# fumiama/Retrieval-based-Voice-Conversion-WebUI

Measured on AMD Instinct MI355X. Metric: real-time factor (audio-sec/wall-sec), 48 kHz v2, 10 s clips, retrieval + NSF-HiFi-GAN decode, higher is better.
Workload: dtype fp16 MFMA operands + fp16 inter-stage streams (ResBlock outputs, ups output of stages 1-3), fp32 accumulate / in-block residual; fp32 MFMA prefilter + fp64 verified IVF distances; 1 GPU; BASELINE configs[1]: v2/48k, 1 x 10 s clip(s) per GPU, T=1198 frames, 599 queries/clip, IVF 10000x768 nlist=256 nprobe=1 k=8 index_rate=0.75; hipgraph=True, index_blob_bytes=32376576, launcher=single process

## Files before the change

retrieval-based-voice-conversion-webui_amd/csrc/nsf.hip:

```cpp
#include <algorithm>
#include <atomic>
#include <cmath>
#include <functional>
#include <memory>
#include <string>
#include <unordered_map>

#include "common.hpp"
#include "nsf_kernels.hpp"
#include "conv_pack.hpp"
#include "rb_stream.hpp"

namespace rvcmi {

thread_local std::string g_last_error;
void set_error(const char* fmt, ...) {
    char buf[1024];
    va_list ap;
    va_start(ap, fmt);
    vsnprintf(buf, sizeof(buf), fmt, ap);
    va_end(ap);
    g_last_error = buf;
}

// ... 133 lines not shown
        s.rb[j].resize(nd);
        for (int m = 0; m < nd; ++m) {
            const int d = cfg->resblock_dilation_sizes[j][m];
            const std::string base = "resblocks." + std::to_string(n);
            const int C = s.cout;
            for (int which = 0; which < 2; ++which) {
                const std::string nm = base + (which ? ".convs2." : ".convs1.") + std::to_string(m);
                const rvcmi_tensor& w = wm.get(nm + ".weight", {C, C, k});
                const rvcmi_tensor& b = wm.get(nm + ".bias", {C});
                const int dil = which ? 1 : d;
                int nt = k, off = -((k * dil - dil) / 2);
                const float* wd = w.data;
                ConvLayer& L2 = which ? s.rb[j][m].second : s.rb[j][m].first;
                build_conv(L2, C, C, 1, &nt, &off, dil,
                           [=](int co, int ci, int, int tap) { return wd[((size_t)co * C + ci) * k + tap]; }, b.data, op);
            }
        }
    }
}

static void nsf_create(const rvcmi_nsf_config* cfg, const rvcmi_tensor* weights, int n_weights, int device, int max_B,
                       int max_T, rvcmi_nsf** out) {
    if (!cfg || !out || (!weights && n_weights)) RVCMI_FAIL(RVCMI_ERR_INVALID, "null argument");
    if (cfg->n_ups < 1 || cfg->n_ups > RVCMI_MAX_UPS || cfg->n_resblock_kernels < 1 ||
        cfg->n_resblock_kernels > RVCMI_MAX_RB)
        RVCMI_FAIL(RVCMI_ERR_INVALID, "bad stage counts");
    if (cfg->operand < 0 || cfg->operand > 2) RVCMI_FAIL(RVCMI_ERR_INVALID, "bad operand type %d", cfg->operand);
    if (max_B < 1 || max_T < 1) RVCMI_FAIL(RVCMI_ERR_INVALID, "max_B/max_T must be positive");
    HIP_CHECK(hipSetDevice(device));
    set_lds_limits();
    rb_stream_prepare();

    std::unique_ptr<rvcmi_nsf> h(new rvcmi_nsf());
    h->opt.load_env({"RB_STREAM", "NO_RB_SPLIT", "POST_DMA", "POST_DBG", "DBG", "Y_F16", "X0_F16", "X0_F16_NOSTREAM"});
    rb_stream_load_env(h->opt);
    h->cfg = *cfg;
    h->device = device;
    h->max_B = max_B;
    h->max_T = max_T;
    const int op = cfg->operand;
    WeightMap wm;
    for (int i = 0; i < n_weights; ++i) wm.m[weights[i].name] = &weights[i];

    const int C0 = cfg->upsample_initial_channel, inter = cfg->inter_channels;
    h->C0 = C0;
    {
        const rvcmi_tensor& w = wm.get("conv_pre.weight", {C0, inter, 7});
        const rvcmi_tensor& b = wm.get("conv_pre.bias", {C0});
        const float* wd = w.data;
        int nt = 7, off = -3;
        build_conv(h->pre, inter, C0, 1, &nt, &off, 1,
                   [=](int co, int ci, int, int tap) { return wd[((size_t)co * inter + ci) * 7 + tap]; }, b.data, op);
    }
    if (cfg->gin_channels) {
        const rvcmi_tensor& w = wm.get("cond.weight", {C0, cfg->gin_channels, 1});
        const rvcmi_tensor& b = wm.get("cond.bias", {C0});
        upload(h->cond_w, std::vector<float>(w.data, w.data + (size_t)C0 * cfg->gin_channels));
        upload(h->cond_b, std::vector<float>(b.data, b.data + C0));
    }
    if (cfg->use_f0) {
        h->lin_w = wm.get("m_source.l_linear.weight", {1, 1}).data[0];
        h->lin_b = wm.get("m_source.l_linear.bias", {1}).data[0];
    }
    int upp = 1;
    for (int i = 0; i < cfg->n_ups; ++i) upp *= cfg->upsample_rates[i];
    h->upp = upp;

// ... 224 lines not shown
#define RBF32_OCC 2
#endif
template <int C> struct RbFullGeom;
#ifndef RBF64_NWV
#define RBF64_NWV 8
#endif
#if RBF64_NWV == 8
template <> struct RbFullGeom<64> { static constexpr int MI = 2, NJ = 2, KG = 4, OCC = 2, NWV = 8; };
#else
template <> struct RbFullGeom<64> { static constexpr int MI = 2, NJ = 3, KG = 4, OCC = 1, NWV = 4; };
#endif
#ifndef RBF32_NWV
#define RBF32_NWV 4
#endif
template <> struct RbFullGeom<32> { static constexpr int MI = 1, NJ = RBF32_NJ, KG = 4, OCC = RBF32_OCC, NWV = RBF32_NWV; };
template <> struct RbFullGeom<16> { static constexpr int MI = 1, NJ = RBF32_NJ, KG = 4, OCC = RBF32_OCC, NWV = RBF32_NWV; };
static int rbf_rows(int C) { return C == 64 ? RbFullGeom<64>::NWV * 32 * RbFullGeom<64>::NJ : RBF32_NWV * 32 * RBF32_NJ; }
template <int C>
constexpr int rbf_nb() { return RbFullGeom<C>::NWV == 8 ? 2 : 3; }
template <typename OpT, int C>
static void launch_rbf_inst(const RbFullArgs& ra, int tiles, int nj, int B, hipStream_t st) {
    using G = RbFullGeom<C>;
    constexpr int R = G::NWV * 32 * G::NJ;
    const size_t smem = (size_t)(R + 2 * RBF_G + R + 2 * RBF_G2) * Tile<C>::STRIDE + 3 * 2 * 32 * G::MI * 4 + 512;
    hipLaunchKernelGGL((k_rb_full<OpT, C, G::MI, G::NJ, G::KG, rbf_nb<C>(), G::OCC, G::NWV>), dim3(tiles, nj, B), dim3(64 * G::NWV), smem, st, ra);
}
constexpr int RBF64S_NJ = 2, RBF64S_NWV = 4, RBF64S_ROWS = RBF64S_NWV * 32 * RBF64S_NJ;
template <typename OpT, int C>
static void launch_rbf_small(const RbFullArgs& ra, int tiles, int nj, int B, hipStream_t st) {
    constexpr int R = RBF64S_ROWS, MI = C == 64 ? 2 : 1, OCCS = C == 64 ? 1 : 2;
    const size_t smem = (size_t)(R + 2 * RBF_G + R + 2 * RBF_G2) * Tile<C>::STRIDE + 3 * 2 * 32 * MI * 4 + 512;
    hipLaunchKernelGGL((k_rb_full<OpT, C, MI, RBF64S_NJ, 4, 3, OCCS, RBF64S_NWV>), dim3(tiles, nj, B), dim3(64 * RBF64S_NWV), smem, st, ra);
}
template <typename OpT>
static void launch_rbf_t(int C, const RbFullArgs& ra, int tiles, int nj, int B, hipStream_t st, bool small64) {
    if (small64 && C == 64) return launch_rbf_small<OpT, 64>(ra, tiles, nj, B, st);
    if (small64 && C == 32) return launch_rbf_small<OpT, 32>(ra, tiles, nj, B, st);
    switch (C) {
        case 64: return launch_rbf_inst<OpT, 64>(ra, tiles, nj, B, st);
        case 32: return launch_rbf_inst<OpT, 32>(ra, tiles, nj, B, st);
        case 16: return launch_rbf_inst<OpT, 16>(ra, tiles, nj, B, st);
        default: RVCMI_FAIL(RVCMI_ERR_INVALID, "fused resblock: unsupported channel count %d", C);
    }
}
template <typename OpT>
static void set_lds_rbf() {
#define RBF_ATTR(C_)                                                                                                        \
    HIP_CHECK(hipFuncSetAttribute(reinterpret_cast<const void*>(&k_rb_full<OpT, C_, RbFullGeom<C_>::MI, RbFullGeom<C_>::NJ, RbFullGeom<C_>::KG, rbf_nb<C_>(), RbFullGeom<C_>::OCC, RbFullGeom<C_>::NWV>), \
                                  hipFuncAttributeMaxDynamicSharedMemorySize, 160 * 1024));
    RBF_ATTR(64) RBF_ATTR(32) RBF_ATTR(16)
    HIP_CHECK(hipFuncSetAttribute(reinterpret_cast<const void*>(&k_rb_full<OpT, 64, 2, RBF64S_NJ, 4, 3, 1, RBF64S_NWV>),
                                  hipFuncAttributeMaxDynamicSharedMemorySize, 160 * 1024));
    HIP_CHECK(hipFuncSetAttribute(reinterpret_cast<const void*>(&k_rb_full<OpT, 32, 1, RBF64S_NJ, 4, 3, 2, RBF64S_NWV>),
                                  hipFuncAttributeMaxDynamicSharedMemorySize, 160 * 1024));
#undef RBF_ATTR
}

static int rb_stream_mode(const rvcmi_nsf* h) {
    if (!h->opt.has("RB_STREAM")) return 2;
    const int v = h->opt.geti("RB_STREAM", 2);
    return v == 0 ? 0 : (v == 1 ? 1 : 2);
}

static bool y_f16(const rvcmi_nsf* h) {
    return h->cfg.operand != RVCMI_OPERAND_F32 && h->opt.geti("Y_F16", 1) != 0;
}

static void run_conv(rvcmi_nsf* h, const ConvLayer& L, ConvArgs a, int B, const char* name, hipStream_t st) {
    if (!a.cf_stride) a.cf_stride = a.Lin;
    a.cin = L.cin;
    a.cout = L.cout;
    a.bias = L.bias.as<float>();
    a.dstep = L.dstep;
    a.nphase = L.nphase;
    const int op = h->cfg.operand;
    int jsum = 0;
    for (int p = 0; p < L.nphase; ++p) {
        a.ph_in_off[p] = L.in_off[p];
        a.ph_ntaps[p] = L.ntaps[p];
        a.ph_w_off[p] = op == RVCMI_OPERAND_F32 ? L.f32_off[p] : L.pack_off[p];
        jsum += L.ntaps[p];
    }
    a.in_off = L.in_off[0];
    const double flops = L.flops_per_pos * (double)a.Lq * B;
    const size_t esz = op == RVCMI_OPERAND_F32 ? 4 : 2;
    double bytes = (double)B * a.Lin * L.cin * (a.in_mode == IN_OP_RAW ? esz : 4) +
                   (double)B * a.Lq * L.nphase * L.cout * (a.out_mode == OUT_ACT ? esz : 4) * (a.accumulate ? 2 : 1) +
                   (a.res ? (double)B * a.Lq * L.nphase * L.cout * 4 : 0) + (double)jsum * L.cin * L.cout * esz;
// ... 143 lines not shown
        fprintf(stderr, "\n");
    }
}


struct Fwd {
    rvcmi_nsf* h;
    int op, B, Te;
    const int* lens;
    const float* har;
    hipStream_t st;
    TapRequest* tr;
    bool want(const char* w) const { return tr && strcmp(tr->what, w) == 0; }
};

struct Act {
    const float* y[3];
    bool half;
    bool raw;
    float div;
    long L;
    int C;
    int lm;
};

using RbLevels = std::vector<std::pair<ConvLayer, ConvLayer>>;

enum class RbPath { F32_CHAIN, SPLIT, STREAM, FULL, PAIR };
struct StagePlan {
    RbPath path;
    bool x0_half;
    bool stage_half;
    bool small64;
};

static float* ydst(rvcmi_nsf* h, size_t j, size_t m) { return (m & 1) ? h->Yb[j].as<float>() : h->Ya[j].as<float>(); }

static size_t max_levels(const Stage& s) {
    size_t n = 0;
    for (const RbLevels& rb : s.rb) n = std::max(n, rb.size());
    return n;
}

static void rb_order(const Stage& s, int* order) {
    const int nk = (int)s.rb.size();
    for (int j = 0; j < nk; ++j) order[j] = j;
    std::sort(order, order + nk, [&](int a, int b) { return s.rb[a][0].first.ntaps[0] > s.rb[b][0].first.ntaps[0]; });
}

static int rbf_halo(const RbLevels& rb) {
    int dsum = 0;
    for (const auto& pr : rb) dsum += pr.first.dstep;
    return (rb[0].first.ntaps[0] - 1) / 2 * (dsum + (int)rb.size());
}

template <typename D>
static void fill_rb_job(D& d, const RbLevels& rb, int m0, int nd, long L, int B, int C, double& flops, double& bytes) {
    d.k = rb[m0].first.ntaps[0];
    d.k_p = rb[m0].first.ntaps_p;
    d.ct1 = rb[m0].first.ct_stride;
    d.ct2 = rb[m0].second.ct_stride;
    for (int m = 0; m < nd; ++m) {
        const ConvLayer& c1 = rb[m0 + m].first;
        const ConvLayer& c2 = rb[m0 + m].second;
        d.w1[m] = c1.w_pack.p;
        d.w2[m] = c2.w_pack.p;
// ... 1 lines not shown
        d.b2[m] = c2.bias.as<float>();
        d.dil[m] = c1.dstep;
        flops += (c1.flops_per_pos + c2.flops_per_pos) * (double)L * B;
        bytes += 2.0 * d.k * C * C * 2;
    }
}

static void stream_jobs(const Fwd& f, const Stage& s, long L, int lm, bool xhalf, bool yhalf, RbStreamDesc* sd, double& flops,
                        double& bytes) {
    rvcmi_nsf* h = f.h;
    const int C = s.cout;
    int order[RVCMI_MAX_RB];
    rb_order(s, order);
    for (size_t oj = 0; oj < s.rb.size(); ++oj) {
        const int j = order[oj];
        RbStreamDesc& d = sd[oj];
        memset(&d, 0, sizeof(d));
        d.src = h->X0.as<float>();
        d.dst = h->Ya[j].as<float>();
        d.y_half = yhalf ? 1 : 0;
        d.x_half = xhalf ? 1 : 0;
        d.lens = f.lens;
        d.lmul = lm;
        fill_rb_job(d, s.rb[j], 0, 3, L, f.B, C, flops, bytes);
        bytes += (double)f.B * L * C * ((yhalf ? 2 : 4) + (xhalf ? 2 : 4));
    }
}

static StagePlan plan_stage(const Fwd& f, const Stage& s, long L, int lm) {
    rvcmi_nsf* h = f.h;
    const int op = f.op, C = s.cout, nk = (int)s.rb.size();
    const bool yh = y_f16(h);
    const bool x0h = yh && h->opt.geti("X0_F16", 1) != 0;
    StagePlan p = {RbPath::PAIR, false, false, false};
    if (op == RVCMI_OPERAND_F32) {
        p.path = RbPath::F32_CHAIN;
        return p;
    }
    const long rows = (long)f.B * L;
    const int mode = rb_stream_mode(h);
    if (((C == 256 && rows <= RB_SPLIT_MAX_ROWS) || (C == 128 && rows <= RB_SPLIT_MAX_ROWS_128)) && nk <= 3 && !h->opt.on("NO_RB_SPLIT") &&
        mode != 1) {
        p.path = RbPath::SPLIT;
        return p;
    }
    bool stream = mode != 0 && nk <= 3 && rb_stream_supported(op, C, 3);
    for (int j = 0; j < nk; ++j) stream = stream && s.rb[j].size() == 3;
    if (stream) {
        auto plans = [&](bool xhalf) {
            RbStreamDesc sd[3];
            double flops = 0, bytes = 0;
            stream_jobs(f, s, L, lm, xhalf, yh, sd, flops, bytes);
            return rb_stream_launch(op, C, 3, sd, nk, (int)L, f.B, L * C, mode == 1, f.st, h->opt, true);
        };
        const bool xh = x0h && !h->opt.on("X0_F16_NOSTREAM") && plans(true);
        if (xh || plans(false)) return {RbPath::STREAM, xh, yh, false};
    }
    if (C <= 64 && max_levels(s) <= 3) {
        p = {RbPath::FULL, x0h, yh, false};
        if (C == 64 || C == 32) {
            long blocks512 = 0;
            for (int j = 0; j < nk; ++j) {
                const int HL = rbf_halo(s.rb[j]);
                blocks512 += (L + (rbf_rows(C) - 2 * HL) - 1) / (rbf_rows(C) - 2 * HL) * f.B;
                if (RBF64S_ROWS - 2 * HL < RBF64S_ROWS / 4) blocks512 = 1 << 30;
            }
            p.small64 = blocks512 < num_cus() / 2 * (C == 64 ? 1 : 2);
        }
    }
    return p;
}

static bool excitation(Fwd& f, int T, const float* f0, const float* noise) {
    rvcmi_nsf* h = f.h;
    const rvcmi_nsf_config& c = h->cfg;
    const int B = f.B, Te = f.Te, upp = h->upp;
    hipStream_t st = f.st;
    const int* lens = f.lens;
    h->prof.launch("phase_scan", 0, (double)B * T * 8, st, [&] {
        hipLaunchKernelGGL(k_phase_scan, dim3(B), dim3(256), 0, st, f0, h->phase.as<float>(), T, (float)c.sr, (float)upp, lens);
    });
    const size_t total = (size_t)B * T * upp;
    h->prof.launch("sine_source", 0, (double)total * (noise ? 8 : 4), st, [&] {
        hipLaunchKernelGGL(k_sine_source, dim3((unsigned)((total + 255) / 256)), dim3(256), 0, st, f0,
                           h->phase.as<float>(), noise, h->har.as<float>(), T, upp, (float)c.sr, h->lin_w, h->lin_b, total);
    });
    f.har = h->har.as<float>();
    if (Te != T) {
        const size_t tot2 = (size_t)B * Te * upp;
        hipLaunchKernelGGL(k_interp_linear, dim3((unsigned)((tot2 + 255) / 256)), dim3(256), 0, st, f.har,
                           h->har2.as<float>(), T * upp, Te * upp, tot2);
        f.har = h->har2.as<float>();
    }
    HIP_CHECK(hipGetLastError());
    if (!f.want("har")) return false;
    TapRequest* tr = f.tr;
    const size_t n = (size_t)B * Te * upp;
    if (n > tr->capacity) RVCMI_FAIL(RVCMI_ERR_NOMEM, "tap capacity");
    HIP_CHECK(hipMemcpyAsync(tr->out_host, f.har, n * 4, hipMemcpyDeviceToHost, st));
    HIP_CHECK(hipStreamSynchronize(st));
// ... 229 lines not shown
        run_conv_jobs(h, L2, a2, nj, f.B, nm, f.st);
    }
}

static void rb_stream(const Fwd& f, const Stage& s, const StagePlan& p, long L, int lm, const float** src) {
    rvcmi_nsf* h = f.h;
    const int C = s.cout, nk = (int)s.rb.size();
    RbStreamDesc sd[3];
    double flops = 0, bytes = 0;
    stream_jobs(f, s, L, lm, p.x0_half, p.stage_half, sd, flops, bytes);
    char nm[48];
    snprintf(nm, sizeof(nm), "rb_stream_c%d", C);
    h->prof.launch(nm, flops, bytes, f.st, [&] {
        rb_stream_launch(f.op, C, 3, sd, nk, (int)L, f.B, L * C, rb_stream_mode(h) == 1, f.st, h->opt);
    });
    HIP_CHECK(hipGetLastError());
    for (int j = 0; j < nk; ++j) src[j] = h->Ya[j].as<float>();
}

static void rb_full(const Fwd& f, const Stage& s, const StagePlan& p, long L, int lm, const float** src) {
    rvcmi_nsf* h = f.h;
    const int C = s.cout, nk = (int)s.rb.size(), B = f.B;
    char nm[48];
    snprintf(nm, sizeof(nm), "rb_full_c%d", C);
    RbFullArgs ra;
    memset(&ra, 0, sizeof(ra));
    ra.L = (int)L;
    ra.lens = f.lens;
    ra.lmul = lm;
    ra.bstride = L * C;
    ra.dbg = dbg_flags(h);
    ra.yh = p.stage_half ? 1 : 0;
    ra.xh = p.x0_half ? 1 : 0;
    const int R = p.small64 ? RBF64S_ROWS : rbf_rows(C);
    int order[RVCMI_MAX_RB];
    rb_order(s, order);
    int max_tiles = 0;
    double flops = 0, bytes = 0;
    for (int oj = 0; oj < nk; ++oj) {
        const int j = order[oj];
        RbFullJob& J = ra.job[oj];
        J.src = h->X0.as<float>();
        J.dst = h->Ya[j].as<float>();
        J.nd = (int)s.rb[j].size();
        fill_rb_job(J, s.rb[j], 0, J.nd, L, B, C, flops, bytes);
        for (int m = 0; m < J.nd; ++m)
            if (J.dil[m] * (J.k - 1) / 2 + J.dil[m] > RBF_G) RVCMI_FAIL(RVCMI_ERR_INVALID, "dilation too large for the fused resblock");
        J.HL = rbf_halo(s.rb[j]);
        J.tvalid = R - 2 * J.HL;
        if (J.tvalid < R / 4) RVCMI_FAIL(RVCMI_ERR_INVALID, "resblock halo too large for the fused kernel");
        J.ntiles = (int)((L + J.tvalid - 1) / J.tvalid);
        max_tiles = std::max(max_tiles, J.ntiles);
        bytes += (double)B * L * C * ((p.stage_half ? 2 : 4) + (p.x0_half ? 2 : 4));
        src[j] = J.dst;
    }
    const size_t nblk = (size_t)max_tiles * nk * B;
    if (ra.dbg & 32) ra.ts = stamp_buffer(h, nblk * 8 * 16, f.st);
    h->prof.launch(nm, flops, bytes, f.st, [&] {
        if (f.op == RVCMI_OPERAND_BF16) launch_rbf_t<__bf16>(C, ra, max_tiles, nk, B, f.st, p.small64);
        else launch_rbf_t<_Float16>(C, ra, max_tiles, nk, B, f.st, p.small64);
    });
    HIP_CHECK(hipGetLastError());
    if (ra.dbg & 32) {
        const int nwv = p.small64 ? RBF64S_NWV : (C == 64 ? RbFullGeom<64>::NWV : RBF32_NWV);
        print_stamps(h, nm, ra, nk, max_tiles, nwv, 16, nblk, f.st);
    }
}

static void rb_pair(const Fwd& f, const Stage& s, long L, int lm, const float** src) {
    rvcmi_nsf* h = f.h;
    const int op = f.op, C = s.cout, nk = (int)s.rb.size(), B = f.B;
    const int mode = rb_stream_mode(h);
    char nm[48], nms[48];
    snprintf(nm, sizeof(nm), "rb_pair_c%d", C);
    snprintf(nms, sizeof(nms), "rb_stream1_c%d", C);
    int order[RVCMI_MAX_RB];
    rb_order(s, order);
    constexpr int NWp = 8;
    for (size_t m = 0; m < max_levels(s); ++m) {
        RbPairArgs ra;
        memset(&ra, 0, sizeof(ra));
        ra.lens = f.lens;
        ra.lmul = lm;
        ra.L = (int)L;
        ra.bstride = L * C;
        ra.dbg = dbg_flags(h);
        RbStreamDesc sd[RVCMI_MAX_RB];
        float* dsts[RVCMI_MAX_RB] = {nullptr};
        int nj = 0, max_tiles = 0, max_rows = 0;
        double flops = 0, bytes = 0;
        for (int oj = 0; oj < nk; ++oj) {
            const int j = order[oj];
            if (m >= s.rb[j].size()) continue;
            RbStreamDesc& d = sd[nj];
            memset(&d, 0, sizeof(d));
            d.src = src[j];
            d.dst = dsts[j] = ydst(h, j, m);
// ... 121 lines not shown

int rvcmi_nsf_create(const rvcmi_nsf_config* cfg, const rvcmi_tensor* weights, int n_weights, int device, int max_B,
                     int max_T, rvcmi_nsf** out) {
    return guarded([&] { nsf_create(cfg, weights, n_weights, device, max_B, max_T, out); });
}
int rvcmi_nsf_destroy(rvcmi_nsf* h) {
    return guarded([&] { delete h; });
}
int rvcmi_nsf_forward(rvcmi_nsf* h, int B, int T, const int* lengths, const float* x, const float* f0, const float* g,
                      const float* noise, int n_res, float* out, void* stream) {
    return guarded([&] { nsf_forward(h, B, T, lengths, x, f0, g, noise, n_res, out, (hipStream_t)stream, nullptr); });
}
int rvcmi_nsf_upp(const rvcmi_nsf* h) { return h ? h->upp : RVCMI_ERR_INVALID; }
size_t rvcmi_nsf_workspace_bytes(const rvcmi_nsf* h) { return h ? h->ws_bytes : 0; }

int rvcmi_nsf_debug_forward(rvcmi_nsf* h, int B, int T, const float* x, const float* f0, const float* g,
                            const float* noise, int n_res, const char* what, float* out_host, size_t capacity_floats,
                            int64_t shape_out[3], void* stream) {
    return guarded([&] {
        if (!what || !out_host || !shape_out) RVCMI_FAIL(RVCMI_ERR_INVALID, "null argument");
        TapRequest tr;
        tr.what = what;
        tr.out_host = out_host;
        tr.capacity = capacity_floats;
        tr.shape = shape_out;
        nsf_forward(h, B, T, nullptr, x, f0, g, noise, n_res, nullptr, (hipStream_t)stream, &tr);
        if (!tr.done) RVCMI_FAIL(RVCMI_ERR_INVALID, "tap '%s' was not produced", what);
    });
}

int rvcmi_nsf_set_option(rvcmi_nsf* h, const char* key, double value) {
    return guarded([&] {
        if (!h || !key) RVCMI_FAIL(RVCMI_ERR_INVALID, "null argument");
        if (!h->opt.set(key, value)) RVCMI_FAIL(RVCMI_ERR_INVALID, "unknown option '%s' for this handle", key);
    });
}
int rvcmi_nsf_profile_enable(rvcmi_nsf* h, int enable) {
    return guarded([&] {
        if (!h) RVCMI_FAIL(RVCMI_ERR_INVALID, "null handle");
        h->prof.enabled = enable != 0;
    });
}
int rvcmi_nsf_profile_read(rvcmi_nsf* h, rvcmi_kernel_stat* stats, int capacity, int* n, int reset) {
    return guarded([&] {
        if (!h) RVCMI_FAIL(RVCMI_ERR_INVALID, "null handle");
        h->prof.read(stats, capacity, n, reset);
    });
}

}
```

retrieval-based-voice-conversion-webui_amd/csrc/nsf_kernels.hpp:

```cpp
#pragma once
#include <hip/hip_runtime.h>

#include "exact_fp.hpp"
#include <stdint.h>

namespace rvcmi {

using bf16x8 = __attribute__((ext_vector_type(8))) __bf16;
using f16x8 = __attribute__((ext_vector_type(8))) _Float16;
using f32x16 = __attribute__((ext_vector_type(16))) float;
using f32x4 = __attribute__((ext_vector_type(4))) float;

__device__ __forceinline__ float lrelu(float v, float slope) { return v > 0.f ? v : v * slope; }

__device__ __forceinline__ int item_rows(const int* __restrict__ lens, int b, int mul, int Lmax) {
    return lens ? max(min(Lmax, lens[b] * mul), min(Lmax, mul)) : Lmax;
}


static __global__ void __launch_bounds__(256) k_phase_scan(const float* __restrict__ f0, float* __restrict__ phase,
                                                   int T, float sr, float upp, const int* __restrict__ lens) {
#pragma clang fp contract(off)
    __shared__ double wsum[4];
    const int b = blockIdx.x;
// ... 636 lines not shown
                    if (a.div_in == 3.f) x = div3_exact(x);
                    else if (a.div_in != 1.f) x = x / a.div_in;
                    v[e] = to_op<OpT>(lrelu(x, a.slope_in));
                }
            } else {
                const float* p = (const float*)a.in + (size_t)b * a.in_bstride + (size_t)(c8 * 8) * a.cf_stride + gr;
#pragma unroll
                for (int e = 0; e < 8; ++e) v[e] = to_op<OpT>(p[(size_t)e * a.cf_stride]);
            }
        }
        *(frag*)(smem + (size_t)r * STRIDE + c8 * 16) = v;
    }
}

template <typename OpT, int MI, int KGROUP, int NB>
__device__ __forceinline__ void conv_load_group(typename Op<OpT>::frag (&Ab)[KGROUP][MI], const OpT* wlane, long ct_stride, int grp) {
    using frag = typename Op<OpT>::frag;
#pragma unroll
    for (int g = 0; g < KGROUP; ++g)
#pragma unroll
        for (int mi = 0; mi < MI; ++mi)
            Ab[g][mi] = *(const frag*)(wlane + (size_t)mi * ct_stride + (size_t)(grp * KGROUP + g) * 512);
}

template <typename OpT, int CIN, int MI, int KGROUP, int NB>
__device__ __forceinline__ void conv_prefetch(typename Op<OpT>::frag (&A)[NB][KGROUP][MI], const OpT* wlane, long ct_stride,
                                              int ntaps_p) {
    const int NG = ntaps_p * Tile<CIN>::CC / KGROUP;
#pragma unroll
    for (int i = 0; i < NB - 1; ++i)
        if (i < NG) conv_load_group<OpT, MI, KGROUP, NB>(A[i], wlane, ct_stride, i);
}

template <typename OpT, int CIN, int MI, int NJ, int KGROUP, int NB>
__device__ __forceinline__ void conv_run(f32x16 (&acc)[MI][NJ], typename Op<OpT>::frag (&A)[NB][KGROUP][MI],
                                         const char* lds_lane, const OpT* wlane, long ct_stride, int ntaps_p, int roff,
                                         int dstep, int dbg = 0) {
    using frag = typename Op<OpT>::frag;
    using TL = Tile<CIN>;
    constexpr int CC = TL::CC;
    constexpr int STRIDE = TL::STRIDE;
    static_assert((CC >= KGROUP) ? (CC % KGROUP == 0) : (KGROUP % CC == 0), "k-group must tile a tap");
    static_assert(NB >= 2 && NB <= 4, "2..4 weight buffers");
    static_assert(KGROUP % 2 == 0, "the B ping-pong needs an even k-group");
    constexpr int GPT = (CC >= KGROUP) ? CC / KGROUP : 1;
    constexpr int TPG = (CC >= KGROUP) ? 1 : KGROUP / CC;
    const int NG = ntaps_p * CC / KGROUP;
    const int dS = dstep * STRIDE;
    (void)dbg;

    auto koff = [&](int k) { return (CC >= KGROUP) ? k * 32 : (k / CC) * dS + (k % CC) * 32; };
    auto readB = [&](frag(&B)[NJ], const char* base, int k) {
        const char* bp = base + koff(k);
#pragma unroll
        for (int jt = 0; jt < NJ; ++jt) B[jt] = *(const frag*)(bp + jt * 32 * STRIDE);
    };

    const char* gb = lds_lane + roff * STRIDE;
    int gi = 0;
    const OpT* an = wlane + (size_t)min(NB - 1, NG - 1) * KGROUP * 512;
    int gn = min(NB - 1, NG - 1);

    frag Bf[2][NJ];
#ifndef RVCMI_KLOOP_V1
#pragma unroll
    for (int jt = 0; jt < NJ; ++jt) {
        Bf[0][jt] = *(const frag*)(gb + koff(0) + jt * 32 * STRIDE);
        __builtin_amdgcn_sched_barrier(0);
    }
#else
    readB(Bf[0], gb, 0);
#endif
    for (int grp = 0; grp < NG; grp += NB) {
#pragma unroll
        for (int u = 0; u < NB; ++u) {
            const int g = grp + u;
            if (g < NG) {
                const char* gbn;
                if constexpr (CC >= KGROUP) gbn = (gi + 1 == GPT) ? gb - (GPT - 1) * KGROUP * 32 + dS : gb + KGROUP * 32;
                else gbn = gb + TPG * dS;
#ifndef RVCMI_KLOOP_V1
#pragma unroll
                for (int k = 0; k < KGROUP; ++k) {
                    const char* nbp = (k + 1 < KGROUP) ? gb + koff(k + 1) : gbn + koff(0);
#pragma unroll
                    for (int mi = 0; mi < MI; ++mi)
#pragma unroll
                        for (int jt = 0; jt < NJ; ++jt) {
                            constexpr int NS = MI * NJ;
                            const int i = mi * NJ + jt;
                            acc[mi][jt] = Op<OpT>::mfma(A[u][k][mi], Bf[k & 1][jt], acc[mi][jt]);
#ifdef RVCMI_KLOOP_ABLATE
                            if (!(RVCMI_KLOOP_ABLATE & 2))
#endif
                            if (i < NJ) Bf[(k + 1) & 1][i] = *(const frag*)(nbp + i * 32 * STRIDE);
#ifdef RVCMI_KLOOP_ABLATE
                            if (!(RVCMI_KLOOP_ABLATE & 1))
#endif
                            if (i >= NS - MI)
                                A[(u + NB - 1) % NB][k][i - (NS - MI)] = *(const frag*)(an + (size_t)(i - (NS - MI)) * ct_stride + k * 512);
                            __builtin_amdgcn_sched_barrier(0);
                        }
                }
#else
#pragma unroll
                for (int k = 0; k < KGROUP; ++k) {
                    if (k + 1 < KGROUP) readB(Bf[(k + 1) & 1], gb, k + 1);
                    else readB(Bf[0], gbn, 0);
#pragma unroll
                    for (int mi = 0; mi < MI; ++mi)
                        A[(u + NB - 1) % NB][k][mi] = *(const frag*)(an + (size_t)mi * ct_stride + k * 512);
#pragma unroll
                    for (int mi = 0; mi < MI; ++mi)
#pragma unroll
                        for (int jt = 0; jt < NJ; ++jt) acc[mi][jt] = Op<OpT>::mfma(A[u][k][mi], Bf[k & 1][jt], acc[mi][jt]);
#pragma unroll
                    for (int i = 0; i < MI * NJ; ++i) {
                        __builtin_amdgcn_sched_group_barrier(0x008, 1, 0);
                        if (i < NJ) __builtin_amdgcn_sched_group_barrier(0x100, 1, 0);
                        else if (i < NJ + MI) __builtin_amdgcn_sched_group_barrier(0x020, 1, 0);
                    }
                }
#endif
                gb = gbn;
                if constexpr (CC >= KGROUP) gi = (gi + 1 == GPT) ? 0 : gi + 1;
                if (gn < NG - 1) {
                    ++gn;
                    an += KGROUP * 512;
                }
            }
        }
    }
}

using lds_cptr_t = const __attribute__((address_space(3))) char*;
__device__ __forceinline__ unsigned lds_address(const void* p) { return (unsigned)(size_t)(lds_cptr_t)p; }
using u32x4_t = __attribute__((ext_vector_type(4))) unsigned;
__device__ __forceinline__ __amdgpu_buffer_rsrc_t weight_rsrc(const void* p) {
    return __builtin_amdgcn_make_buffer_rsrc((void*)p, 0, 0x7fffffff, 0x00020000);
}
template <typename OpT>
__device__ __forceinline__ typename Op<OpT>::frag weight_load(__amdgpu_buffer_rsrc_t r, unsigned voff, unsigned soff) {
    return __builtin_bit_cast(typename Op<OpT>::frag, __builtin_amdgcn_raw_buffer_load_b128(r, voff, soff, 0));
}
template <typename OpT, int MI>
__device__ __forceinline__ void kconv_prefetch(typename Op<OpT>::frag (&A)[8][MI], __amdgpu_buffer_rsrc_t r, unsigned loff, unsigned ctb) {
#pragma unroll
    for (int kk = 0; kk < 8; ++kk)
#pragma unroll
        for (int mi = 0; mi < MI; ++mi) A[kk][mi] = weight_load<OpT>(r, loff + kk * 1024, mi * ctb);
}
template <typename OpT, int CIN, int MI, int NJ, int STRIDE>
__device__ __forceinline__ void kconv(f32x16 (&acc)[MI][NJ], typename Op<OpT>::frag (&A)[8][MI], unsigned lds_row, __amdgpu_buffer_rsrc_t r,
                                      unsigned loff, unsigned ctb, int ntaps, int dstep) {
    using frag = typename Op<OpT>::frag;
    constexpr int CC = CIN / 16, GPT = CC / 8;
    static_assert(CIN % 128 == 0, "kconv: C_in must be a multiple of 128");
    constexpr unsigned TS = 32u * STRIDE;
    auto ld = [](unsigned a) { return *(const __attribute__((address_space(3))) frag*)(size_t)a; };
    frag Bf[2][NJ];
#pragma unroll
    for (int jt = 0; jt < NJ; ++jt) {
        Bf[0][jt] = ld(lds_row + jt * TS);
        __builtin_amdgcn_sched_barrier(0);
    }
// ... 830 lines not shown
        char* og = (char*)a.out + ((size_t)b * a.out_bstride + (size_t)q0 * a.u * a.cout) * esz;
        for (int i = threadIdx.x; i < nrows * cpr; i += 256) {
            const int row = i / cpr, c = i - row * cpr;
            *(uint4*)(og + ((size_t)row * cpr + c) * 16) = *(const uint4*)(ot + (size_t)row * pitch + c * 16);
        }
    }
}

struct RbFullJob {
    const float* src;
    float* dst;
    const void* w1[3];
    const void* w2[3];
    const float* b1[3];
    const float* b2[3];
    long ct1, ct2;
    int k, k_p;
    int dil[3];
    int nd;
    int HL;
    int tvalid;
    int ntiles;
};
struct RbFullArgs {
    RbFullJob job[3];
    int L;
    const int* lens;
    int lmul;
    long bstride;
    int dbg;
    int yh;
    int xh;
    unsigned long long* ts;
};

constexpr int RBF_G = 32;
constexpr int RBF_G2 = 8;

template <typename OpT, int C, int MI, int NJ, int KG, int NB, int OCC = 1, int NWV = 4>
static __global__ void __launch_bounds__(64 * NWV, OCC) k_rb_full(RbFullArgs a) {
    constexpr int NT = 64 * NWV;
    using TL = Tile<C>;
    constexpr int STRIDE = TL::STRIDE;
    constexpr int SLAB = 32 * NJ;
    constexpr int R = NWV * SLAB;
    constexpr int XROWS = R + 2 * RBF_G;
    constexpr int HROWS = R + 2 * RBF_G2;
    constexpr int CP = 32 * MI;
    extern __shared__ __attribute__((aligned(16))) char smem[];
    char* X = smem;
    char* H = smem + (size_t)XROWS * STRIDE;
    float* bias_l = (float*)(smem + (size_t)(XROWS + HROWS) * STRIDE);
    unsigned long long* tsl = (unsigned long long*)(bias_l + 3 * 2 * CP);

    const RbFullJob& J = a.job[blockIdx.y];
    if ((int)blockIdx.x >= J.ntiles) return;
    const int b = blockIdx.z;
    const int Lb = item_rows(a.lens, b, a.lmul, a.L);
    const int tg0 = blockIdx.x * J.tvalid - J.HL;
    if (tg0 + J.HL >= Lb) return;
    const float* src = J.src + (size_t)b * a.bstride;
    float* dst = J.dst + (size_t)b * a.bstride;
    const int wave = threadIdx.x >> 6, lane = threadIdx.x & 63;
    const int slab = wave * SLAB;
    const int half4 = 4 * (lane >> 5);

// ... 131 lines not shown
    {
        constexpr int W = STRIDE / 16;
        const uint4 z = make_uint4(0, 0, 0, 0);
        for (int i = threadIdx.x; i < 2 * RBF_G * W; i += NT) {
            const int r = i / W, c = i - r * W;
            const int row = r < RBF_G ? r : RBF_G + R + (r - RBF_G);
            *(uint4*)(X + (size_t)row * STRIDE + c * 16) = z;
        }
        for (int i = threadIdx.x; i < 2 * RBF_G2 * W; i += NT) {
            const int r = i / W, c = i - r * W;
            const int row = r < RBF_G2 ? r : RBF_G2 + R + (r - RBF_G2);
            *(uint4*)(H + (size_t)row * STRIDE + c * 16) = z;
        }
        for (int i = threadIdx.x; i < J.nd * 2 * CP; i += NT) {
            const int m = i / (2 * CP), w = (i / CP) & 1, c = i % CP;
            const float* bp = w ? J.b2[m] : J.b1[m];
            bias_l[i] = c < C ? bp[c] : 0.f;
        }
    }

    stamp();
    typename Op<OpT>::frag A[NB][KG][MI];
    conv_prefetch<OpT, C, MI, KG, NB>(A, (const OpT*)J.w1[0] + lane * 8, J.ct1, J.k_p);
    char* xw = X + (size_t)(RBF_G + slab + (lane & 31)) * STRIDE + half4 * 2;
    char* hw = H + (size_t)(RBF_G2 + slab + (lane & 31)) * STRIDE + half4 * 2;
    publish_operand<OpT, C, MI, NJ, STRIDE, false>(xw, xacc, rowmask);
    stamp();
    __syncthreads();
    stamp();

    const char* xl = X + (size_t)(slab + (lane & 31)) * STRIDE + (lane >> 5) * 16;
    const char* hl = H + (size_t)(slab + (lane & 31)) * STRIDE + (lane >> 5) * 16;
    const int p2 = (J.k - 1) / 2;

    for (int m = 0; m < J.nd; ++m) {
        const int p1 = J.dil[m] * (J.k - 1) / 2;
        f32x16 hacc[MI][NJ];
        {
            const float* bl = bias_l + (m * 2 + 0) * CP + half4;
#pragma unroll
            for (int mi = 0; mi < MI; ++mi)
#pragma unroll
                for (int g = 0; g < 4; ++g) {
                    const f32x4 bv = *(const f32x4*)(bl + mi * 32 + 8 * g);
#pragma unroll
                    for (int jt = 0; jt < NJ; ++jt)
#pragma unroll
                        for (int e = 0; e < 4; ++e) hacc[mi][jt][4 * g + e] = bv[e];
                }
        }
        conv_run<OpT, C, MI, NJ, KG, NB>(hacc, A, xl, (const OpT*)J.w1[m] + lane * 8, J.ct1, J.k_p, RBF_G - p1, J.dil[m], a.dbg);
        conv_prefetch<OpT, C, MI, KG, NB>(A, (const OpT*)J.w2[m] + lane * 8, J.ct2, J.k_p);
        if (m == 0) stamp();
        if (interior) publish_operand<OpT, C, MI, NJ, STRIDE, false>(hw, hacc, rowmask);
        else publish_operand<OpT, C, MI, NJ, STRIDE, true>(hw, hacc, rowmask);
        if (m == 0) stamp();
        __syncthreads();
        if (m == 0) stamp();
        {
            const float* bl = bias_l + (m * 2 + 1) * CP + half4;
#pragma unroll
            for (int mi = 0; mi < MI; ++mi)
#pragma unroll
                for (int g = 0; g < 4; ++g) {
                    const f32x4 bv = *(const f32x4*)(bl + mi * 32 + 8 * g);
#pragma unroll
                    for (int jt = 0; jt < NJ; ++jt)
#pragma unroll
                        for (int e = 0; e < 4; ++e) xacc[mi][jt][4 * g + e] += bv[e];
                }
        }
        conv_run<OpT, C, MI, NJ, KG, NB>(xacc, A, hl, (const OpT*)J.w2[m] + lane * 8, J.ct2, J.k_p, RBF_G2 - p2, 1, a.dbg);
        if (m + 1 < J.nd) conv_prefetch<OpT, C, MI, KG, NB>(A, (const OpT*)J.w1[m + 1] + lane * 8, J.ct1, J.k_p);
        if (m == 0) stamp();
        if (m + 1 < J.nd) {
            if (interior) publish_operand<OpT, C, MI, NJ, STRIDE, false>(xw, xacc, rowmask);
            else publish_operand<OpT, C, MI, NJ, STRIDE, true>(xw, xacc, rowmask);
            if (m == 0) stamp();
            __syncthreads();
            if (m == 0) stamp();
        }
    }
    stamp();

    if (a.yh) {
        _Float16* dsth = (_Float16*)J.dst + (size_t)b * a.bstride;
        if constexpr (TIO) {
            constexpr int TSH = C * 2 + 16;
            constexpr int C8 = C / 8;
            __syncthreads();
#pragma unroll
            for (int mi = 0; mi < MI; ++mi)
#pragma unroll
                for (int jt = 0; jt < NJ; ++jt)
#pragma unroll
                    for (int g = 0; g < 4; ++g)
                        *(uint2*)(smem + (size_t)(slab + jt * 32 + (lane & 31)) * TSH + (mi * 32 + 8 * g + half4) * 2) =
                            pack4_h(xacc[mi][jt][4 * g + 0], xacc[mi][jt][4 * g + 1], xacc[mi][jt][4 * g + 2], xacc[mi][jt][4 * g + 3]);
            __syncthreads();
            if (!(a.dbg & 16)) {
                const int nrow = min(R - 2 * J.HL, Lb - (tg0 + J.HL));
                const int tot = nrow * C8;
                for (int i = threadIdx.x; i < tot; i += NT) {
                    const int r = i / C8, c8 = i - r * C8;
                    const int row = J.HL + r;
// ... 69 lines not shown
```

Baseline: 5592 x real-time (audio-sec/wall-sec), whole job.

## Add tall 768-row fused resblock tile for C=32 and skip padded taps

Adds a new launch configuration for the fused ResBlock kernel at 32 channels: 8 waves, NJ=3, 768 rows per block. The planner picks it automatically when blocks are plentiful relative to the CU count, cutting halo recomputation per tile. The k-loop now exits early past the real tap count when taps are padded to a k-group multiple, skipping MFMA work on zero-padded weights. Risks include lower occupancy, higher LDS use, and a goto inside an unrolled loop that may hurt scheduling.

```diff
diff --git a/retrieval-based-voice-conversion-webui_amd/csrc/nsf.hip b/retrieval-based-voice-conversion-webui_amd/csrc/nsf.hip
--- a/retrieval-based-voice-conversion-webui_amd/csrc/nsf.hip
+++ b/retrieval-based-voice-conversion-webui_amd/csrc/nsf.hip
@@ -189,7 +189,7 @@
     rb_stream_prepare();
 
     std::unique_ptr<rvcmi_nsf> h(new rvcmi_nsf());
-    h->opt.load_env({"RB_STREAM", "NO_RB_SPLIT", "POST_DMA", "POST_DBG", "DBG", "Y_F16", "X0_F16", "X0_F16_NOSTREAM"});
+    h->opt.load_env({"RB_STREAM", "NO_RB_SPLIT", "POST_DMA", "POST_DBG", "RBF_PAD_TAP", "RBF32_TALL", "DBG", "Y_F16", "X0_F16", "X0_F16_NOSTREAM"});
     rb_stream_load_env(h->opt);
     h->cfg = *cfg;
     h->device = device;
@@ -480,8 +480,16 @@
     const size_t smem = (size_t)(R + 2 * RBF_G + R + 2 * RBF_G2) * Tile<C>::STRIDE + 3 * 2 * 32 * MI * 4 + 512;
     hipLaunchKernelGGL((k_rb_full<OpT, C, MI, RBF64S_NJ, 4, 3, OCCS, RBF64S_NWV>), dim3(tiles, nj, B), dim3(64 * RBF64S_NWV), smem, st, ra);
 }
+constexpr int RBF32T_NJ = 3, RBF32T_NWV = 8, RBF32T_NB = 3, RBF32T_ROWS = RBF32T_NWV * 32 * RBF32T_NJ;
 template <typename OpT>
-static void launch_rbf_t(int C, const RbFullArgs& ra, int tiles, int nj, int B, hipStream_t st, bool small64) {
+static void launch_rbf_tall(const RbFullArgs& ra, int tiles, int nj, int B, hipStream_t st) {
+    constexpr int R = RBF32T_ROWS;
+    const size_t smem = (size_t)(R + 2 * RBF_G + R + 2 * RBF_G2) * Tile<32>::STRIDE + 3 * 2 * 32 * 4 + 1024;
+    hipLaunchKernelGGL((k_rb_full<OpT, 32, 1, RBF32T_NJ, 4, RBF32T_NB, 1, RBF32T_NWV>), dim3(tiles, nj, B), dim3(64 * RBF32T_NWV), smem, st, ra);
+}
+template <typename OpT>
+static void launch_rbf_t(int C, const RbFullArgs& ra, int tiles, int nj, int B, hipStream_t st, bool small64, bool tall32) {
+    if (tall32 && C == 32) return launch_rbf_tall<OpT>(ra, tiles, nj, B, st);
     if (small64 && C == 64) return launch_rbf_small<OpT, 64>(ra, tiles, nj, B, st);
     if (small64 && C == 32) return launch_rbf_small<OpT, 32>(ra, tiles, nj, B, st);
     switch (C) {
@@ -501,7 +509,15 @@
                                   hipFuncAttributeMaxDynamicSharedMemorySize, 160 * 1024));
     HIP_CHECK(hipFuncSetAttribute(reinterpret_cast<const void*>(&k_rb_full<OpT, 32, 1, RBF64S_NJ, 4, 3, 2, RBF64S_NWV>),
                                   hipFuncAttributeMaxDynamicSharedMemorySize, 160 * 1024));
+    HIP_CHECK(hipFuncSetAttribute(reinterpret_cast<const void*>(&k_rb_full<OpT, 32, 1, RBF32T_NJ, 4, RBF32T_NB, 1, RBF32T_NWV>),
+                                  hipFuncAttributeMaxDynamicSharedMemorySize, 160 * 1024));
 #undef RBF_ATTR
+}
+
+static int rbf32_tall_mode(const rvcmi_nsf* h) {
+    if (!h->opt.has("RBF32_TALL")) return 2;
+    const int v = h->opt.geti("RBF32_TALL", 2);
+    return v == 0 ? 0 : (v == 1 ? 1 : 2);
 }
 
 static int rb_stream_mode(const rvcmi_nsf* h) {
@@ -711,6 +727,7 @@
     bool x0_half;
     bool stage_half;
     bool small64;
+    bool tall32;
 };
 
 static float* ydst(rvcmi_nsf* h, size_t j, size_t m) { return (m & 1) ? h->Yb[j].as<float>() : h->Ya[j].as<float>(); }
@@ -778,7 +795,7 @@
     const int op = f.op, C = s.cout, nk = (int)s.rb.size();
     const bool yh = y_f16(h);
     const bool x0h = yh && h->opt.geti("X0_F16", 1) != 0;
-    StagePlan p = {RbPath::PAIR, false, false, false};
+    StagePlan p = {RbPath::PAIR, false, false, false, false};
     if (op == RVCMI_OPERAND_F32) {
         p.path = RbPath::F32_CHAIN;
         return p;
@@ -800,18 +817,26 @@
             return rb_stream_launch(op, C, 3, sd, nk, (int)L, f.B, L * C, mode == 1, f.st, h->opt, true);
         };
         const bool xh = x0h && !h->opt.on("X0_F16_NOSTREAM") && plans(true);
-        if (xh || plans(false)) return {RbPath::STREAM, xh, yh, false};
+        if (xh || plans(false)) return {RbPath::STREAM, xh, yh, false, false};
     }
     if (C <= 64 && max_levels(s) <= 3) {
-        p = {RbPath::FULL, x0h, yh, false};
+        p = {RbPath::FULL, x0h, yh, false, false};
         if (C == 64 || C == 32) {
-            long blocks512 = 0;
+            long blocks512 = 0, blocks768 = 0;
+            bool fits768 = true;
             for (int j = 0; j < nk; ++j) {
                 const int HL = rbf_halo(s.rb[j]);
                 blocks512 += (L + (rbf_rows(C) - 2 * HL) - 1) / (rbf_rows(C) - 2 * HL) * f.B;
                 if (RBF64S_ROWS - 2 * HL < RBF64S_ROWS / 4) blocks512 = 1 << 30;
+                blocks768 += (L + (RBF32T_ROWS - 2 * HL) - 1) / (RBF32T_ROWS - 2 * HL) * f.B;
+                fits768 = fits768 && RBF32T_ROWS - 2 * HL >= RBF32T_ROWS / 4;
             }
             p.small64 = blocks512 < num_cus() / 2 * (C == 64 ? 1 : 2);
+            if (C == 32 && fits768) {
+                const int tall = rbf32_tall_mode(h);
+                p.tall32 = tall == 1 || (tall == 2 && !p.small64 && blocks768 >= 4L * num_cus());
+                if (p.tall32) p.small64 = false;
+            }
         }
     }
     return p;
@@ -1107,7 +1132,8 @@
     ra.dbg = dbg_flags(h);
     ra.yh = p.stage_half ? 1 : 0;
     ra.xh = p.x0_half ? 1 : 0;
-    const int R = p.small64 ? RBF64S_ROWS : rbf_rows(C);
+    ra.pad_tap = h->opt.geti("RBF_PAD_TAP", 0) != 0 ? 1 : 0;
+    const int R = p.tall32 ? RBF32T_ROWS : (p.small64 ? RBF64S_ROWS : rbf_rows(C));
     int order[RVCMI_MAX_RB];
     rb_order(s, order);
     int max_tiles = 0;
@@ -1132,12 +1158,12 @@
     const size_t nblk = (size_t)max_tiles * nk * B;
     if (ra.dbg & 32) ra.ts = stamp_buffer(h, nblk * 8 * 16, f.st);
     h->prof.launch(nm, flops, bytes, f.st, [&] {
-        if (f.op == RVCMI_OPERAND_BF16) launch_rbf_t<__bf16>(C, ra, max_tiles, nk, B, f.st, p.small64);
-        else launch_rbf_t<_Float16>(C, ra, max_tiles, nk, B, f.st, p.small64);
+        if (f.op == RVCMI_OPERAND_BF16) launch_rbf_t<__bf16>(C, ra, max_tiles, nk, B, f.st, p.small64, p.tall32);
+        else launch_rbf_t<_Float16>(C, ra, max_tiles, nk, B, f.st, p.small64, p.tall32);
     });
     HIP_CHECK(hipGetLastError());
     if (ra.dbg & 32) {
-        const int nwv = p.small64 ? RBF64S_NWV : (C == 64 ? RbFullGeom<64>::NWV : RBF32_NWV);
+        const int nwv = p.tall32 ? RBF32T_NWV : (p.small64 ? RBF64S_NWV : (C == 64 ? RbFullGeom<64>::NWV : RBF32_NWV));
         print_stamps(h, nm, ra, nk, max_tiles, nwv, 16, nblk, f.st);
     }
 }
@@ -1325,6 +1351,8 @@
 int rvcmi_nsf_set_option(rvcmi_nsf* h, const char* key, double value) {
     return guarded([&] {
         if (!h || !key) RVCMI_FAIL(RVCMI_ERR_INVALID, "null argument");
+        if ((!strcmp(key, "RBF_PAD_TAP") || !strcmp(key, "RBF32_TALL")) && value == value && value != 0.0 && value != 1.0)
+            RVCMI_FAIL(RVCMI_ERR_INVALID, "option '%s' takes 0 or 1", key);
         if (!h->opt.set(key, value)) RVCMI_FAIL(RVCMI_ERR_INVALID, "unknown option '%s' for this handle", key);
     });
 }
diff --git a/retrieval-based-voice-conversion-webui_amd/csrc/nsf_kernels.hpp b/retrieval-based-voice-conversion-webui_amd/csrc/nsf_kernels.hpp
--- a/retrieval-based-voice-conversion-webui_amd/csrc/nsf_kernels.hpp
+++ b/retrieval-based-voice-conversion-webui_amd/csrc/nsf_kernels.hpp
@@ -692,10 +692,10 @@
         if (i < NG) conv_load_group<OpT, MI, KGROUP, NB>(A[i], wlane, ct_stride, i);
 }
 
-template <typename OpT, int CIN, int MI, int NJ, int KGROUP, int NB>
+template <typename OpT, int CIN, int MI, int NJ, int KGROUP, int NB, bool REAL = false>
 __device__ __forceinline__ void conv_run(f32x16 (&acc)[MI][NJ], typename Op<OpT>::frag (&A)[NB][KGROUP][MI],
                                          const char* lds_lane, const OpT* wlane, long ct_stride, int ntaps_p, int roff,
-                                         int dstep, int dbg = 0) {
+                                         int dstep, int dbg = 0, int nks = 0) {
     using frag = typename Op<OpT>::frag;
     using TL = Tile<CIN>;
     constexpr int CC = TL::CC;
@@ -708,6 +708,7 @@
     const int NG = ntaps_p * CC / KGROUP;
     const int dS = dstep * STRIDE;
     (void)dbg;
+    (void)nks;
 
     auto koff = [&](int k) { return (CC >= KGROUP) ? k * 32 : (k / CC) * dS + (k % CC) * 32; };
     auto readB = [&](frag(&B)[NJ], const char* base, int k) {
@@ -742,6 +743,8 @@
 #ifndef RVCMI_KLOOP_V1
 #pragma unroll
                 for (int k = 0; k < KGROUP; ++k) {
+                    if constexpr (REAL && TPG > 1)
+                        if (k > 0 && k % CC == 0 && g * KGROUP + k >= nks) goto done;
                     const char* nbp = (k + 1 < KGROUP) ? gb + koff(k + 1) : gbn + koff(0);
 #pragma unroll
                     for (int mi = 0; mi < MI; ++mi)
@@ -791,6 +794,7 @@
             }
         }
     }
+done:;
 }
 
 using lds_cptr_t = const __attribute__((address_space(3))) char*;
@@ -1687,6 +1691,7 @@
     int yh;
     int xh;
     unsigned long long* ts;
+    int pad_tap;
 };
 
 constexpr int RBF_G = 32;
@@ -1884,6 +1889,8 @@
     const char* xl = X + (size_t)(slab + (lane & 31)) * STRIDE + (lane >> 5) * 16;
     const char* hl = H + (size_t)(slab + (lane & 31)) * STRIDE + (lane >> 5) * 16;
     const int p2 = (J.k - 1) / 2;
+    constexpr bool REAL = TL::CC < KG;
+    const int nks = (REAL && !a.pad_tap ? J.k : J.k_p) * TL::CC;
 
     for (int m = 0; m < J.nd; ++m) {
         const int p1 = J.dil[m] * (J.k - 1) / 2;
@@ -1901,7 +1908,7 @@
                         for (int e = 0; e < 4; ++e) hacc[mi][jt][4 * g + e] = bv[e];
                 }
         }
-        conv_run<OpT, C, MI, NJ, KG, NB>(hacc, A, xl, (const OpT*)J.w1[m] + lane * 8, J.ct1, J.k_p, RBF_G - p1, J.dil[m], a.dbg);
+        conv_run<OpT, C, MI, NJ, KG, NB, REAL>(hacc, A, xl, (const OpT*)J.w1[m] + lane * 8, J.ct1, J.k_p, RBF_G - p1, J.dil[m], a.dbg, nks);
         conv_prefetch<OpT, C, MI, KG, NB>(A, (const OpT*)J.w2[m] + lane * 8, J.ct2, J.k_p);
         if (m == 0) stamp();
         if (interior) publish_operand<OpT, C, MI, NJ, STRIDE, false>(hw, hacc, rowmask);
@@ -1922,7 +1929,7 @@
                         for (int e = 0; e < 4; ++e) xacc[mi][jt][4 * g + e] += bv[e];
                 }
         }
-        conv_run<OpT, C, MI, NJ, KG, NB>(xacc, A, hl, (const OpT*)J.w2[m] + lane * 8, J.ct2, J.k_p, RBF_G2 - p2, 1, a.dbg);
+        conv_run<OpT, C, MI, NJ, KG, NB, REAL>(xacc, A, hl, (const OpT*)J.w2[m] + lane * 8, J.ct2, J.k_p, RBF_G2 - p2, 1, a.dbg, nks);
         if (m + 1 < J.nd) conv_prefetch<OpT, C, MI, KG, NB>(A, (const OpT*)J.w1[m + 1] + lane * 8, J.ct1, J.k_p);
         if (m == 0) stamp();
         if (m + 1 < J.nd) {
```

Measured after the change: 5693 x real-time (audio-sec/wall-sec), whole job, median of 6. 1.02x the previous value.
